# VishnoiAman777/FedRec-with-PytorchDistributed

Hardware: AMD Instinct MI355X
Metric: impressions/sec/node per FedAvg round + MIND AUC, 8 client-GPUs (higher is better)
Workload: dtype bf16

## Files before the change

### fedrec_with_pytorchdistributed_amd/csrc/bind_text_head.cpp

```cpp
#include "binding_util.h"

namespace {

int64_t head_titles(const at::Tensor& table, const OptTensor& ids, int64_t T) {
  check_dev(table, "table");
  TORCH_CHECK(table.dim() == 2 && table.is_contiguous() && table.scalar_type() == at::kBFloat16,
              "fedrec::head: table [rows, D] contiguous bf16");
  TORCH_CHECK(T >= 1 && table.size(0) % T == 0, "fedrec::head: table rows not a multiple of T");
  if (ids.has_value()) {
    check_dev(*ids, "ids");
    TORCH_CHECK(ids->dim() == 1 && ids->is_contiguous() && ids->scalar_type() == at::kInt, "fedrec::head: ids int32 [U]");
    return ids->size(0);
  }
  return table.size(0) / T;
}

Tensor2 head_score(const at::Tensor& table, const OptTensor& ids, int64_t T, const at::Tensor& w1, const at::Tensor& b1,
                   const at::Tensor& w2, const at::Tensor& b2, bool store_e, const OptTensor& nreal) {
  const int64_t U = head_titles(table, ids, T), D = table.size(1), Q = w1.size(0);
  check_dev(w1, "w1");
  TORCH_CHECK(w1.scalar_type() == at::kBFloat16 && w1.is_contiguous() && w1.size(1) == D, "fedrec::head_score: w1 bf16 [Q, D]");
  TORCH_CHECK(b1.scalar_type() == at::kFloat && w2.scalar_type() == at::kFloat && b2.scalar_type() == at::kFloat &&
                  b1.numel() == Q && w2.numel() == Q && b2.numel() == 1 && b1.is_contiguous() && w2.is_contiguous() &&
                  b1.is_cuda() && w2.is_cuda() && b2.is_cuda(),
              "fedrec::head_score: b1 / w2 [Q], b2 [1] fp32 device");
  TORCH_CHECK(fr_head_supported((int)D, (int)Q, (int)T), "fedrec::head_score: unsupported shape D=", D, " Q=", Q, " T=", T);
  const c10::DeviceGuard g(table.device());
  auto e = store_e ? at::empty({U * T, Q}, table.options()) : at::empty({0}, table.options());
  const int slices = fr_head_score_slices((int)Q);
  auto a = slices > 1 ? at::empty({slices, U * T}, table.options().dtype(at::kFloat))
                      : at::empty({U * T}, table.options().dtype(at::kFloat));
  check_rc(fr_head_score(table.data_ptr(), opt_int_ptr(ids), (int)U, (int)T, (int)D, (int)Q, w1.data_ptr(),
                         b1.data_ptr<float>(), w2.data_ptr<float>(), b2.data_ptr<float>(),
                         store_e ? e.data_ptr() : nullptr, a.data_ptr<float>(), opt_nreal(nreal, table), cur_stream()),
           "head_score");
  return {e, a};
}

Tensor3 head_pool(const at::Tensor& table, const OptTensor& ids, int64_t T, const at::Tensor& a, const OptTensor& tokens,
                  const OptTensor& nreal, bool want_bf16) {
  const int64_t U = head_titles(table, ids, T), D = table.size(1);
  check_dev(a, "a");
  TORCH_CHECK(a.scalar_type() == at::kFloat && (a.numel() == U * T || (a.dim() == 2 && a.size(0) == 2 && a.size(1) == U * T)) &&
                  a.is_contiguous(),
              "fedrec::head_pool: a [U*T] (or [2, U*T] score partials) fp32");
  if (tokens.has_value()) {
    check_dev(*tokens, "tokens");
    TORCH_CHECK(tokens->scalar_type() == at::kInt && tokens->dim() == 3 && tokens->size(1) == 2 &&
                    tokens->size(2) == T && tokens->is_contiguous() && tokens->size(0) * T >= table.size(0),
                "fedrec::head_pool: tokens int32 [N, 2, T] covering the table");
  }
  const c10::DeviceGuard g(table.device());
  auto pooled = at::empty({U, D}, a.options());
  auto alpha = at::empty({U, T}, a.options());
  auto pooled_b = at::empty({want_bf16 ? U : 0, D}, a.options().dtype(at::kBFloat16));
  check_rc(fr_head_pool(table.data_ptr(), opt_int_ptr(ids), a.data_ptr<float>(), a.dim() == 2 ? (int)a.size(0) : 1,
                        opt_int_ptr(tokens), (int)U, (int)T, (int)D, pooled.data_ptr<float>(), alpha.data_ptr<float>(),
                        opt_nreal(nreal, table), cur_stream(), want_bf16 ? pooled_b.data_ptr() : nullptr),
           "head_pool");
  return {pooled, alpha, pooled_b};
}

Tensor2 head_pool_bwd(const at::Tensor& table, const OptTensor& ids, int64_t T, const at::Tensor& alpha,
                      const at::Tensor& g, const OptTensor& nreal) {
  const int64_t U = head_titles(table, ids, T), D = table.size(1);
  check_dev(alpha, "alpha");
  check_dev(g, "g");
  TORCH_CHECK(alpha.scalar_type() == at::kFloat && alpha.numel() == U * T && alpha.is_contiguous() &&
                  g.scalar_type() == at::kFloat && g.numel() == U * D && g.is_contiguous(),
              "fedrec::head_pool_bwd: alpha [U, T], g [U, D] fp32");
  const c10::DeviceGuard dg(table.device());
  auto da = at::empty({U * T}, alpha.options());
  auto db2p = at::empty({std::max<int64_t>(U, 1)}, alpha.options());
  check_rc(fr_head_pool_bwd(table.data_ptr(), opt_int_ptr(ids), alpha.data_ptr<float>(), g.data_ptr<float>(), (int)U,
                            (int)T, (int)D, da.data_ptr<float>(), db2p.data_ptr<float>(), opt_nreal(nreal, table),
                            cur_stream()),
           "head_pool_bwd");
  return {da, db2p};
}

Tensor4 head_wgrad(const at::Tensor& table, const OptTensor& ids, int64_t T, const at::Tensor& e, const at::Tensor& da,
                   const at::Tensor& w2, const at::Tensor& db2p, const OptTensor& nreal) {
  const int64_t U = head_titles(table, ids, T), D = table.size(1), Q = w2.numel();
  check_dev(e, "e");
  check_dev(da, "da");
  check_dev(w2, "w2");
  check_dev(db2p, "db2p");
  TORCH_CHECK(e.scalar_type() == at::kBFloat16 && e.is_contiguous() && e.numel() == U * T * Q,
              "fedrec::head_wgrad: e bf16 [U*T, Q]");
  TORCH_CHECK(da.scalar_type() == at::kFloat && da.numel() == U * T && w2.scalar_type() == at::kFloat &&
                  w2.is_contiguous() && db2p.scalar_type() == at::kFloat && db2p.numel() >= U,
              "fedrec::head_wgrad: da / w2 / db2p");
  TORCH_CHECK(fr_head_supported((int)D, (int)Q, (int)T), "fedrec::head_wgrad: unsupported shape");
  const c10::DeviceGuard g(table.device());
  auto fopt = da.options();
  auto dW1 = at::empty({Q, D}, fopt);
  auto small = at::empty({2 * Q + 1}, fopt);
  float* db1 = small.data_ptr<float>();
  float* dw2 = db1 + Q;
  float* db2 = dw2 + Q;
  auto run = [&](float* scratch, const int* nr) {
    return fr_head_wgrad(e.data_ptr(), table.data_ptr(), opt_int_ptr(ids), da.data_ptr<float>(), db2p.data_ptr<float>(),
                         w2.data_ptr<float>(), (int)U, (int)T, (int)D, (int)Q, dW1.data_ptr<float>(), db1, dw2, db2,
                         scratch, nr, cur_stream());
  };
  const long need = run(nullptr, nullptr);
  TORCH_CHECK(need > 0, "fedrec::head_wgrad: unsupported shape");
  auto scratch = at::empty({need}, fopt);
  check_rc((int)run(scratch.data_ptr<float>(), opt_nreal(nreal, table)), "head_wgrad");
  return {dW1, small.narrow(0, 0, Q), small.narrow(0, Q, Q), small.narrow(0, 2 * Q, 1)};
}

Tensor3 head_pool_bwd_g(const at::Tensor& table, const OptTensor& ids, int64_t T, const at::Tensor& alpha,
                        const at::Tensor& g, at::Tensor e, const OptTensor& nreal) {
  const int64_t U = head_titles(table, ids, T), D = table.size(1);
  check_dev(alpha, "alpha");
  check_dev(g, "g");
  check_dev(e, "e");
  TORCH_CHECK(alpha.scalar_type() == at::kFloat && alpha.numel() == U * T && alpha.is_contiguous() &&
                  g.scalar_type() == at::kFloat && g.numel() == U * D && g.is_contiguous(),
              "fedrec::head_pool_bwd_g: alpha [U, T], g [U, D] fp32");
  TORCH_CHECK(e.scalar_type() == at::kBFloat16 && e.is_contiguous() && U > 0 && e.numel() % (U * T) == 0,
              "fedrec::head_pool_bwd_g: e bf16 [U*T, Q]");
  const int64_t Q = U > 0 ? e.numel() / (U * T) : 0;
  TORCH_CHECK(fr_head_g_supported((int)D, (int)Q, (int)T), "fedrec::head_pool_bwd_g: unsupported shape");
  const c10::DeviceGuard dg(table.device());
  auto da = at::empty({U * T}, alpha.options());
  auto db2p = at::empty({std::max<int64_t>(U, 1)}, alpha.options());
// ... 167 lines not shown
```

### fedrec_with_pytorchdistributed_amd/csrc/launchers.h

```cpp
#pragma once
#include <hip/hip_runtime_api.h>

extern "C" {

void fr_gemm_set_variant(int v);
int fr_gemm_nt_bf16(const void* A, const void* W, const float* bias, const void* R, void* C, int M, int N, int K, int act,
                    int c_rows, hipStream_t s);
int fr_gemm_nt_bf16_split(const void* A, const void* W, const float* bias, void* C, int M, int N, int K, int c_rows,
                          const int* full_rows, int n_partial, hipStream_t s);
int fr_gemm_gelu_bwd_colpart(const void* A, const void* W, const void* Z, void* C, float* colpart, int M, int N, int K,
                             int c_rows, hipStream_t s);
int fr_gemm_nt_bf16_dual(const void* A, const void* W, const float* bias, void* C, void* Z, int M, int N, int K,
                         int c_rows, hipStream_t s);

long fr_wgrad_bf16(const void* dY, const void* X, float* C, float* scratch, int M, int N, int K, int accumulate,
                   hipStream_t s);

void fr_ln_set_wide(int v);
int fr_layer_norm_bf16(const void* x, const float* w, const float* b, void* y, int rows, int D, float eps,
                       const void* res, hipStream_t s);
int fr_layer_norm_scatter_bf16(const void* x, const float* w, const float* b, void* y, int rows, int D, float eps,
                               const void* res, const int* dst, hipStream_t s);
int fr_layer_norm_bwd_bf16(const void* x, const float* w, const void* dy, void* dx, float* dw, float* db, int rows, int D,
                           float eps, hipStream_t s, float* dxs, void* dxz, float pdrop, unsigned long long seed,
                           unsigned long long offset);
int fr_gelu_bf16(const void* z, const void* dh, void* out, long n, int bwd, hipStream_t s);
int fr_embed_ln_bf16(const int* tokens, const void* word, const void* pos, const float* w, const float* b, void* y,
                     int rows, int D, int T, float eps, hipStream_t s);
int fr_embed_ln_rows_bf16(const int* tokens, const int* src, const void* word, const void* pos, const float* w,
                          const float* b, void* y, int rows, int D, int T, float eps, hipStream_t s);

int fr_dropout_add_bf16(const void* h, const void* res, void* out, long n, float p, unsigned long long seed,
                        unsigned long long offset, hipStream_t s);

void fr_title_attn_set_waves(int w);
int fr_title_attention_bf16(const void* qkv, const int* mask, void* out, int n_titles, int T, int H, int D,
                            hipStream_t s);
int fr_title_attention_drop_bf16(const void* qkv, const int* mask, void* out, int n_titles, int T, int H, int D,
                                 float pdrop, unsigned long long seed, unsigned long long offset, hipStream_t s);
int fr_title_plan(const int* mask, int n, int T, int* rowmap, int* src, int* kv_start, int* kv_len, int* qstart,
                  int* n_kv, hipStream_t s);
int fr_title_attention_packed_bf16(const void* qkv, const int* rowmap, const int* kv_start, const int* kv_len,
                                   const int* qstart, void* out, int n_titles, int T, int H, int D, hipStream_t s);

void fr_title_attn_bwd_set_variant(int v);
int fr_title_attention_bwd_bf16(const void* qkv, const void* dout, const int* mask, void* dqkv, int n_titles, int T, int H,
                                int D, hipStream_t s);
int fr_title_attention_bwd_drop_bf16(const void* qkv, const void* dout, const int* mask, void* dqkv, int n_titles,
                                     int T, int H, int D, float pdrop, unsigned long long seed,
                                     unsigned long long offset, hipStream_t s);

int fr_title_attention_long_bf16(const void* qkv, const int* mask, void* out, int n_titles, int T, int H, int D,
                                 hipStream_t s);
int fr_title_attention_bwd_long_bf16(const void* qkv, const void* dout, const int* mask, void* dqkv, int n_titles,
                                     int T, int H, int D, hipStream_t s);

int fr_colsum_chunks();
int fr_colsum_bf16(const void* x, int M, int N, float* partial, float* out, hipStream_t s, int ld);
int fr_gelu_bwd_colsum_bf16(const void* df, const void* z, void* dz, int M, int N, float* partial, float* out,
                            hipStream_t s);
int fr_embed_grad_bf16(const void* dx, const int* sorted, const int* perm, int R, int D, float* dword, int* scratch,
                       hipStream_t s);

void fr_head_score_set_rows(int r);
void fr_head_score_set_ilv(int v);
void fr_head_wgrad_g_set_kt(int kt);
int fr_head_supported(int D, int Q, int T);
int fr_head_g_supported(int D, int Q, int T);
int fr_head_score_slices(int Q);
int fr_head_score(const void* table, const int* ids, int U, int T, int D, int Q, const void* W1, const float* b1,
                  const float* w2, const float* b2, void* e_out, float* a_out, const int* nreal, hipStream_t s);
int fr_head_pool(const void* table, const int* ids, const float* a, int slices, const int* tokens, int U, int T, int D,
                 float* pooled, float* alpha, const int* nreal, hipStream_t s, void* pooled_b);
int fr_head_pool_bwd(const void* table, const int* ids, const float* alpha, const float* g, int U, int T, int D,
                     float* da, float* db2p, const int* nreal, hipStream_t s);
long fr_head_wgrad(const void* e, const void* table, const int* ids, const float* da, const float* db2p,
                   const float* w2, int U, int T, int D, int Q, float* dW1, float* db1, float* dw2, float* db2,
                   float* scratch, const int* nreal, hipStream_t s);
int fr_head_pool_bwd_g(const void* table, const int* ids, const float* alpha, const float* g, int U, int T, int D,
                       int Q, float* da, float* db2p, void* e, float* cs, const int* nreal, hipStream_t s);
long fr_head_wgrad_g(const void* G, const void* table, const int* ids, const float* cs, const float* db2p,
                     const float* w2, int U, int T, int D, int Q, float* dW1, float* db1, float* dw2, float* db2,
                     float* scratch, const int* nreal, hipStream_t s, const void* pend, int pend_cblocks,
                     int pend_total);

int fr_additive_pool_fwd(const void* x, const void* e, const float* w2, const float* b2, float* out, float* alpha,
                         int n, int T, int D, int Q, int is_bf16, const int* keep, hipStream_t s);
int fr_additive_pool_rows(int T, int D, int Q, int is_bf16);
int fr_additive_pool_bwd(const void* x, const void* e, const float* alpha, const float* w2, const float* g, float* dx,
                         void* dpre, float* dw2, float* db2, float* dsum, int n, int T, int D, int Q, int R,
                         int is_bf16, hipStream_t s);
int fr_upool_bwd_da(const float* x, const float* e, const float* alpha, const float* w2, const float* g, float* dx,
                    float* dpre, float* da8, int n, int T, int D, int Q, hipStream_t s, void* dpre_b);

int fr_user_attn_fwd(const float* qkv, float* ctx, float* stats, int B, int H, int NH, int dk, const int* keep,
                     hipStream_t s, void* ctx_b);
int fr_user_qkv_attn_fwd(const void* xd, const void* W, const float* bias, int Din, float* qkv, float* ctx,
                         float* stats, int B, int H, int NH, int dk, const int* keep, hipStream_t s, void* ctx_b);
int fr_user_attn_bwd_dctx(const float* qkv, const float* stats, const float* dctx, void* dqkv, const void* dpre,
                          const void* w1t, int Qd, int B, int H, int NH, int dk, const int* keep, hipStream_t s);
int fr_user_attn_bwd(const float* qkv, const float* stats, const float* dctx, void* dqkv, int B, int H, int NH,
                     int dk, const int* keep, hipStream_t s, int out_bf16);

void fr_score_set_variant(int v);
int fr_score_ce(const float* cand, const float* user, float* loss, float* scores, float* dcand, float* duser, int B,
                int C, int D, int sigm, const int* ci, float* loss_total, hipStream_t s);
int fr_user_pool_score(const float* x, const float* e, const float* w2, const float* b2, const int* keep,
                       const float* cand, const int* ci, int B, int T, int D, int Q, int C, int sigm, float* lossb,
                       float* scores, float* dcand, float* loss_total, float* dctx, float* dpre, void* dpre_b,
                       float* da8, hipStream_t s);

void fr_segsum_set_variant(int v);
void fr_segsum_set_ldp_block(int v);
int fr_segsum_chunks(int R);
int fr_segment_sum_rows(const float* rows, const int* perm, const int* seg_ptr, const int* inv, float* out, int U, int D,
                        int R, float* scratch, hipStream_t s, int zero_empty);
int fr_segment_sum_rows_ldp(const float* rows, const int* perm, const int* seg_ptr, const int* inv, float* out, int U,
                            int D, int R, float* scratch, float clip, float noise_std, unsigned long long seed,
                            unsigned long long offset, const unsigned long long* dev_off, hipStream_t s);
int fr_ldp_rows(const float* rows, float* out, int R, int D, float clip, float noise_std, unsigned long long seed,
                unsigned long long offset, hipStream_t s, const unsigned long long* dev_off);

void fr_small_gemm_set_rd(int v);
void fr_small_gemm_set_defer(int on);
long fr_small_gemm(const void* const* ptrs, const int* ints, const float* floats, const unsigned long long* seeds,
                   const unsigned long long* dev_off, int n, float* scratch, int tile, hipStream_t s);
int fr_small_gemm_has_pending();
int fr_small_gemm_batch_bytes();
int fr_small_gemm_take_pending(void* dst, int dst_bytes, int* c_blocks, int* total);
int fr_small_gemm_flush_pending(hipStream_t s);
long fr_colsum_f32(const float* const* xs, float* const* outs, const int* ints, int n, float* part, hipStream_t s);
int fr_gather_dropout(const float* v, const int* idx, void* out, int out_bf16, int M, int K, float p,
                      unsigned long long seed, unsigned long long offset, const unsigned long long* dev_off,
                      hipStream_t s);

int fr_adam_flat(float* p, const float* g, float* m, float* v, void* plow, long n, float lr, float b1, float b2,
                 float omb1, float omb2, float eps, float bc1, float bc2, float grad_scale, hipStream_t s);
int fr_adam_dev(float* p, float* g, float* m, float* v, void* plow, long n, float lr, double b1, double b2, float omb1,
                float omb2, float eps, float grad_scale, const long long* step, const float* loss, float* ring,
                int ring_n, hipStream_t s, int nseg, const float* const* gsrc, const long* goff, const long* gn,
                const int* skip);
int fr_multi_cast(const float* const* src, void* const* dst, const long* n, const int* to_bf16, int nseg,
                  long long* bump, hipStream_t s, long long* bump2, const long* nsrc, const int* fill, int ntseg,
                  const float* const* tsrc, void* const* tdst, const int* tR, const int* tC, const int* tld);
int fr_multi_cast_t(const float* const* src, void* const* dst, const int* R, const int* C, const int* ld, int nseg,
                    hipStream_t s);

int fr_sample_batch(const int* rows, const int* pos, const long long* neg_ptr, const int* negs, const long long* his_ptr,
                    const int* his, int* cand, int* hout, int B, int npr, int H, int truncate, unsigned long long seed,
                    unsigned long long offset, int valid, hipStream_t s);
int fr_dedup(const int* ids, int R, int num_news, int* uniq, int* inv, int* perm, int* seg_ptr, int* u_count,
             hipStream_t s);
int fr_multi_copy(const int* const* src, int* const* dst, const long* nsrc, const long* ndst, const int* fill, int n,
                  hipStream_t s);

void fr_topk_set_splits(int s);
int fr_topk_splits(long B, long N);
int fr_topk_scores(const float* user, const float* table, const int* exclude, void* ws, float* scores, int* ids, long B,
                   long N, int D, long E, int k, int min_id, hipStream_t s);

int fr_secagg_mask(const float* x, int* out, long n, float scale, float clipv, const unsigned long long* seeds,
                   const int* signs, int npeers, unsigned long long round, hipStream_t s);
int fr_secagg_unmask(const int* x, float* out, long n, float inv_scale, hipStream_t s);
int fr_secagg_hist(const float* x, long n, unsigned* scratch, int* out, const unsigned long long* seeds,
                   const int* signs, int npeers, unsigned long long round, hipStream_t s);
int fr_secagg_mask_exact(const float* x, int* out, long n, const int* H, int W, const unsigned long long* seeds,
                         const int* signs, int npeers, unsigned long long round, hipStream_t s);
// ... 13 lines not shown
```

### fedrec_with_pytorchdistributed_amd/csrc/text_head.hip

```cpp
#include "common.h"
#include "launchers.h"
#include "gemm_batch.h"

#include <stdlib.h>
#include <string.h>

#include <algorithm>

namespace {

constexpr int MAXT = 128;

__device__ __forceinline__ float tanh_fast(float x) {
  const float e = __builtin_amdgcn_exp2f(x * 2.8853900817779268f);
  return 1.0f - 2.0f * __builtin_amdgcn_rcpf(1.0f + e);
}

__device__ __attribute__((aligned(16))) bf16 g_zero_row[512];
__device__ float g_zero_f32[64];

__device__ __forceinline__ const bf16* hrow(const bf16* __restrict__ table, const int* __restrict__ ids, int m, int T,
                                            int D) {
  const int u = m / T;
  const int t = m - u * T;
// ... 146 lines not shown
      }
      if constexpr (SW) {
        static_assert(QFW <= 8, "lgkmcnt staging");
        __builtin_amdgcn_s_setprio(1);
#pragma unroll
        for (int i = 0; i < QFW; ++i) {
          lgkm_tie_rt(QFW - 1 - i, wr[i]);
          if (i == 0) {
#pragma unroll
            for (int j = 0; j < RFW; ++j) asm volatile("" : "+v"(xr[j]));
          }
#pragma unroll
          for (int j = 0; j < RFW; ++j)
            acc[i][j] = __builtin_amdgcn_mfma_f32_16x16x32_bf16(__builtin_bit_cast(bf16x8, wr[i]),
                                                                __builtin_bit_cast(bf16x8, xr[j]), acc[i][j], 0, 0, 0);
          if constexpr (ILV) {
            const int pc_ = kk * QFW + i;
            if (pc_ < PPW && nxt) issue_one(pc_, nst, nk0);
          }
        }
        __builtin_amdgcn_s_setprio(0);
        continue;
      }
      asm volatile("s_waitcnt lgkmcnt(0)" ::: "memory");
#pragma unroll
      for (int j = 0; j < RFW; ++j) asm volatile("" : "+v"(xr[j]));
#pragma unroll
      for (int i = 0; i < QFW; ++i) asm volatile("" : "+v"(wr[i]));
      __builtin_amdgcn_s_setprio(1);
#pragma unroll
      for (int i = 0; i < QFW; ++i)
#pragma unroll
        for (int j = 0; j < RFW; ++j)
          acc[i][j] = __builtin_amdgcn_mfma_f32_16x16x32_bf16(__builtin_bit_cast(bf16x8, wr[i]),
                                                              __builtin_bit_cast(bf16x8, xr[j]), acc[i][j], 0, 0, 0);
      __builtin_amdgcn_s_setprio(0);
    }
  }
  __syncthreads();

  float part[RFW];
#pragma unroll
  for (int j = 0; j < RFW; ++j) part[j] = 0.f;
#pragma unroll
  for (int i = 0; i < QFW; i += 2) {
    float v[2][RFW][4];
#pragma unroll
    for (int h = 0; h < 2; ++h) {
      const int qb = wq * QFW * 16 + (i + h) * 16 + fq * 4;
      const float4 bb = *(const float4*)(b1 + qb);
      const float4 ww = *(const float4*)(w2 + qb);
#pragma unroll
      for (int j = 0; j < RFW; ++j) {
        v[h][j][0] = tanh_fast(acc[i + h][j][0] + bb.x);
        v[h][j][1] = tanh_fast(acc[i + h][j][1] + bb.y);
        v[h][j][2] = tanh_fast(acc[i + h][j][2] + bb.z);
        v[h][j][3] = tanh_fast(acc[i + h][j][3] + bb.w);
        part[j] += v[h][j][0] * ww.x + v[h][j][1] * ww.y + v[h][j][2] * ww.z + v[h][j][3] * ww.w;
      }
    }
    if (e_out != nullptr) {
#pragma unroll
      for (int j = 0; j < RFW; ++j) {
        const int m = m0 + wm * 16 * RFW + j * 16 + fr;
        store_pair16_if(e_out + (size_t)(m < M ? m : 0) * ldq + wq * QFW * 16 + i * 16, v[0][j], v[1][j], fq, m < M);
      }
    }
  }
  float* red = (float*)smem;
#pragma unroll
  for (int j = 0; j < RFW; ++j) {
    const float s = group4_sum(part[j]);
    if (fq == 0) red[wq * MR + wm * 16 * RFW + j * 16 + fr] = s;
  }
  __syncthreads();
  if (tid < MR && m0 + tid < M) {
    float sa;
    if constexpr (WQ == 4) sa = (red[tid] + red[MR + tid]) + (red[2 * MR + tid] + red[3 * MR + tid]);
    else sa = red[tid] + red[MR + tid];
    a_out[m0 + tid] = sa + b2v;
  }
}

template <int TPT>
__global__ __launch_bounds__(384) void head_pool2_kernel(const bf16* __restrict__ table, const int* __restrict__ ids,
                                                         const float* __restrict__ a, const float* __restrict__ a2,
                                                         const int* __restrict__ tokens,
                                                         int T, int D, float* __restrict__ pooled,
                                                         float* __restrict__ alpha, const int* __restrict__ nreal,
                                                         bf16* __restrict__ pooled_b) {
  __shared__ float part[3072];
  const int u = blockIdx.x, tid = threadIdx.x, lane = tid & 63, wave = tid >> 6;
  if (nreal != nullptr && u >= nreal[0]) {
    for (int d = tid; d < D; d += blockDim.x) {
      pooled[(size_t)u * D + d] = 0.f;
      if (pooled_b != nullptr) pooled_b[(size_t)u * D + d] = f2bf(0.f);
    }
    for (int t = tid; t < T; t += blockDim.x) alpha[(size_t)u * T + t] = 0.f;
    return;
  }
  const int id = ids != nullptr ? ids[u] : u;
  const bf16* xe = table + (size_t)id * T * D;
  const int DC = D >> 3, TG = 384 / DC;
  const int dc = tid % DC, tgr = tid / DC;
  const int tg = tgr < TG ? tgr : TG - 1;
  bf16x8 v[TPT];
#pragma unroll
  for (int i = 0; i < TPT; ++i) {
    const int t = tg + TG * i;
    v[i] = *(const bf16x8*)(xe + (size_t)(t < T ? t : T - 1) * D + dc * 8);
  }
  float av[2], m = -INFINITY;
  bool keep[2];
#pragma unroll
  for (int c = 0; c < 2; ++c) {
    const int t = lane + 64 * c;
    keep[c] = t < T && (tokens == nullptr || tokens[((size_t)id * 2 + 1) * T + t] != 0);
    av[c] = keep[c] ? (a2 != nullptr ? a[(size_t)u * T + t] + a2[(size_t)u * T + t] : a[(size_t)u * T + t]) : -INFINITY;
    m = fmaxf(m, av[c]);
  }
  m = wave_max(m);
  if (!(m > -INFINITY)) m = 0.f;
  float p[2], l = 0.f;
#pragma unroll
  for (int c = 0; c < 2; ++c) {
    p[c] = keep[c] ? __expf(av[c] - m) : 0.f;
    l += p[c];
  }
  const float inv = 1.0f / (wave_sum(l) + 1e-8f * __expf(-m));
  const float al0 = p[0] * inv, al1 = p[1] * inv;
  if (wave == 0) {
    if (lane < T) alpha[(size_t)u * T + lane] = al0;
    if (lane + 64 < T) alpha[(size_t)u * T + lane + 64] = al1;
  }
  float acc[8] = {0.f, 0.f, 0.f, 0.f, 0.f, 0.f, 0.f, 0.f};
#pragma unroll
  for (int i = 0; i < TPT; ++i) {
    const int t = tg + TG * i;
    const float w0 = __shfl(al0, t & 63, 64), w1 = __shfl(al1, t & 63, 64);
    const float w = t < T ? (t < 64 ? w0 : w1) : 0.f;
    if (t < T) {
#pragma unroll
      for (int k = 0; k < 8; ++k) acc[k] += w * (float)v[i][k];
    }
  }
  if (tgr < TG) {
#pragma unroll
    for (int k = 0; k < 8; ++k) part[tg * D + dc * 8 + k] = acc[k];
  }
  __syncthreads();
  for (int d = tid; d < D; d += 384) {
    float s = 0.f;
    for (int j = 0; j < TG; ++j) s += part[j * D + d];
    pooled[(size_t)u * D + d] = s;
    if (pooled_b != nullptr) pooled_b[(size_t)u * D + d] = f2bf(s);
  }
}

template <int TPW>
__global__ __launch_bounds__(384) void head_pool_bwd2_kernel(const bf16* __restrict__ table,
                                                             const int* __restrict__ ids,
                                                             const float* __restrict__ alpha,
                                                             const float* __restrict__ g, int T, int D,
                                                             float* __restrict__ da, float* __restrict__ db2p,
                                                             const int* __restrict__ nreal) {
  __shared__ float dal[MAXT];
  const int u = blockIdx.x, tid = threadIdx.x, lane = tid & 63, wave = tid >> 6;
  if (nreal != nullptr && u >= nreal[0]) {
    for (int t = tid; t < T; t += blockDim.x) da[(size_t)u * T + t] = 0.f;
    if (tid == 0) db2p[u] = 0.f;
    return;
  }
  const int id = ids != nullptr ? ids[u] : u;
  const bf16* xe = table + (size_t)id * T * D;
  const float* gu = g + (size_t)u * D;
  const int DC = D >> 3;
  bf16x8 v[TPW][2];
#pragma unroll
  for (int i = 0; i < TPW; ++i) {
    const int t = wave + 6 * i;
    const bf16* row = xe + (size_t)(t < T ? t : T - 1) * D;
#pragma unroll
    for (int c = 0; c < 2; ++c) {
      const int dc = lane + 64 * c;
      v[i][c] = *(const bf16x8*)(row + (dc < DC ? dc : 0) * 8);
    }
  }
  float gv[2][8];
#pragma unroll
  for (int c = 0; c < 2; ++c) {
    const int dc = lane + 64 * c;
    const float4 g0 = dc < DC ? *(const float4*)(gu + dc * 8) : make_float4(0.f, 0.f, 0.f, 0.f);
    const float4 g1 = dc < DC ? *(const float4*)(gu + dc * 8 + 4) : make_float4(0.f, 0.f, 0.f, 0.f);
    gv[c][0] = g0.x; gv[c][1] = g0.y; gv[c][2] = g0.z; gv[c][3] = g0.w;
    gv[c][4] = g1.x; gv[c][5] = g1.y; gv[c][6] = g1.z; gv[c][7] = g1.w;
  }
  float s[TPW];
#pragma unroll
  for (int i = 0; i < TPW; ++i) {
    s[i] = 0.f;
#pragma unroll
// ... 703 lines not shown
  for (int j = 0; j < 4; ++j) xo[j] = G_BYTES + tr_off_pitch(2 * GKT, r0, wk * 64 + j * 16, q, p);
#pragma unroll
  for (int i = 0; i < QF; ++i) yo[i] = tr_off_pitch(2 * GQT, r0, wq * QF * 16 + i * 16, q, p);
  for (int st = 0; st < nsteps; ++st) {
    const int left = nsteps - 1 - st;
    const int inflight = left < NSTAGE - 2 ? left : NSTAGE - 2;
    __builtin_amdgcn_sched_barrier(0);
    if (inflight >= 2) asm volatile("s_waitcnt vmcnt(8) lgkmcnt(0)\n\ts_barrier" ::: "memory");
    else if (inflight == 1) asm volatile("s_waitcnt vmcnt(4) lgkmcnt(0)\n\ts_barrier" ::: "memory");
    else asm volatile("s_waitcnt vmcnt(0) lgkmcnt(0)\n\ts_barrier" ::: "memory");
    __builtin_amdgcn_sched_barrier(0);
    const bool nxt = st + NSTAGE - 1 < nsteps;
    const int nbuf = (st + NSTAGE - 1) % NSTAGE;
    if (nxt) stage(nbuf, mb + (st + NSTAGE - 1) * WTM);
    const uint32_t base = lds0 + (st % NSTAGE) * GSTB;
    s16x4 xr[8];
#pragma unroll
    for (int j = 0; j < 4; ++j) tr_read2<4 * 2 * GKT>(base + xo[j], xr[2 * j], xr[2 * j + 1]);
    s16x4 yr[2][4];
    tr_read2<4 * 2 * GQT>(base + yo[0], yr[0][0], yr[0][1]);
    tr_read2<4 * 2 * GQT>(base + yo[1], yr[0][2], yr[0][3]);
    bf16x8 xb[4];
#pragma unroll
    for (int ip = 0; ip < QF / 2; ++ip) {
      const int cur = ip & 1;
      if (ip + 1 < QF / 2) {
        tr_read2<4 * 2 * GQT>(base + yo[2 * ip + 2], yr[cur ^ 1][0], yr[cur ^ 1][1]);
        tr_read2<4 * 2 * GQT>(base + yo[2 * ip + 3], yr[cur ^ 1][2], yr[cur ^ 1][3]);
        lgkm_tie4<4>(yr[cur]);
      } else {
        lgkm_tie4<0>(yr[cur]);
      }
      if (ip == 0) {
        asm volatile("" : "+v"(xr[0]), "+v"(xr[1]), "+v"(xr[2]), "+v"(xr[3]), "+v"(xr[4]), "+v"(xr[5]), "+v"(xr[6]),
                     "+v"(xr[7]));
#pragma unroll
        for (int j = 0; j < 4; ++j) xb[j] = join(xr[2 * j], xr[2 * j + 1]);
      }
      __builtin_amdgcn_sched_barrier(0);
      __builtin_amdgcn_s_setprio(1);
#pragma unroll
      for (int f = 0; f < 2; ++f) {
        const bf16x8 ya = join(yr[cur][2 * f], yr[cur][2 * f + 1]);
#pragma unroll
        for (int j = 0; j < 4; ++j)
          acc[2 * ip + f][j] = __builtin_amdgcn_mfma_f32_16x16x32_bf16(xb[j], ya, acc[2 * ip + f][j], 0, 0, 0);
      }
      __builtin_amdgcn_s_setprio(0);
      __builtin_amdgcn_sched_barrier(0);
    }
  }
  float* out = P + (size_t)s * Q * D;
#pragma unroll
  for (int i = 0; i < QF; ++i) {
    const int qq2 = wq * QF * 16 + i * 16 + (lane & 15);
#pragma unroll
    for (int j = 0; j < 4; ++j) {
      const int k = k0 + wk * 64 + j * 16 + 4 * g;
      *(f32x4*)(out + (size_t)qq2 * D + k) = acc[i][j];
    }
  }
  const int per = (2 * Q + tiles_k - 1) / tiles_k;
  const int c = kt * per + tid;
  if (tid < per && c < 2 * Q) {
    const int which = c / Q, qc = c - which * Q;
    const float* src = cs + ((size_t)which * U) * Q + qc;
    float a0 = 0.f, a1 = 0.f, a2 = 0.f, a3 = 0.f;
    int u = u_lo;
    for (; u + 3 < u_hi; u += 4) {
      a0 += src[(size_t)u * Q];
      a1 += src[(size_t)(u + 1) * Q];
      a2 += src[(size_t)(u + 2) * Q];
      a3 += src[(size_t)(u + 3) * Q];
    }
    for (; u < u_hi; ++u) a0 += src[(size_t)u * Q];
    (which == 0 ? dw2p : dsump)[(size_t)s * Q + qc] = (a0 + a1) + (a2 + a3);
  }
}

int g_cus = 0;
int g_score_ilv = 1;
int g_score_rows = 0;

}

extern "C" void fr_head_score_set_rows(int r) { g_score_rows = r; }
extern "C" void fr_head_score_set_ilv(int v) { g_score_ilv = v; }

extern "C" int fr_head_supported(int D, int Q, int T) {
  return D % 256 == 0 && D <= 1024 && (Q == 128 || Q == 256 || Q == 384) && T >= 1 && T <= MAXT &&
         (T + 384 / (D / 8) - 1) / (384 / (D / 8)) <= 32;
}

extern "C" int fr_head_score(const void* table, const int* ids, int U, int T, int D, int Q, const void* W1,
                             const float* b1, const float* w2, const float* b2, void* e_out, float* a_out,
                             const int* nreal, hipStream_t s) {
  if (!fr_head_supported(D, Q, T)) return 1;
  const int M = U * T;
  if (M == 0) return 0;
  if (Q == 384) {
    if (g_cus == 0) {
      int dev = 0;
      (void)hipGetDevice(&dev);
      (void)hipDeviceGetAttribute(&g_cus, hipDeviceAttributeMultiprocessorCount, dev);
      if (g_cus <= 0) g_cus = 256;
    }
    const long Me = nreal != nullptr ? std::max<long>((long)M - 64L * T, (long)T) : (long)M;
    const long rounds192 = ((Me + 191) / 192 + g_cus - 1) / g_cus, rounds160 = ((Me + 159) / 160 + g_cus - 1) / g_cus;
    const bool r160 = g_score_rows == 160 || (g_score_rows == 0 && rounds160 * (160 + 384) < rounds192 * (192 + 384));
#define LAUNCH_S2(RF_, IL_)                                                                                  \
  hipLaunchKernelGGL((head_score2_kernel<6, RF_, 64, 2, 4, true, IL_>), dim3((M + 32 * RF_ - 1) / (32 * RF_)),     \
                     dim3(512), 0, s, (const bf16*)table, ids, M, T, D, (const bf16*)W1, b1, w2, b2, (bf16*)e_out, \
                     a_out, Q, nreal)
    if (r160) {
      if (g_score_ilv) LAUNCH_S2(5, true);
      else LAUNCH_S2(5, false);
    } else {
      if (g_score_ilv) LAUNCH_S2(6, true);
      else LAUNCH_S2(6, false);
    }
#undef LAUNCH_S2
    return 0;
  }
  if (Q == 256)
    hipLaunchKernelGGL((head_score2_kernel<4, 4, 64, 2, 4, true>), dim3((M + 127) / 128), dim3(512), 0, s,
                       (const bf16*)table, ids, M, T, D, (const bf16*)W1, b1, w2, b2, (bf16*)e_out, a_out, Q, nreal);
  else
    hipLaunchKernelGGL((head_score2_kernel<2, 4, 64, 2, 4, true>), dim3((M + 127) / 128), dim3(512), 0, s,
                       (const bf16*)table, ids, M, T, D, (const bf16*)W1, b1, w2, b2, (bf16*)e_out, a_out, Q, nreal);
  return 0;
}

extern "C" int fr_head_score_slices(int Q) {
  (void)Q;
  return 1;
}

extern "C" int fr_head_pool(const void* table, const int* ids, const float* a, int slices, const int* tokens, int U,
                            int T, int D, float* pooled, float* alpha, const int* nreal, hipStream_t s,
                            void* pooled_b) {
  const float* a2 = slices == 2 ? a + (size_t)U * T : nullptr;
  if (T > MAXT || D % 8 != 0 || D / 8 > 384) return 1;
  if (U == 0) return 0;
  const int TG = 384 / (D / 8), tpt = (T + TG - 1) / TG;
  if (tpt > 32) return 1;
  {
#define LAUNCH_POOL2(N)                                                                                          \
  hipLaunchKernelGGL(head_pool2_kernel<N>, dim3(U), dim3(384), 0, s, (const bf16*)table, ids, a, a2, tokens, T, D, \
                     pooled, alpha, nreal, (bf16*)pooled_b)
    if (tpt <= 13) LAUNCH_POOL2(13);
    else if (tpt <= 16) LAUNCH_POOL2(16);
    else LAUNCH_POOL2(32);
#undef LAUNCH_POOL2
    return 0;
  }
  return 0;
}

extern "C" int fr_head_pool_bwd(const void* table, const int* ids, const float* alpha, const float* g, int U, int T,
                                int D, float* da, float* db2p, const int* nreal, hipStream_t s) {
  if (T > MAXT || D % 8 != 0 || D / 8 > 128) return 1;
  if (U == 0) return 0;
  const int tpw = (T + 5) / 6;
  {
#define LAUNCH_PBWD2(N)                                                                                           \
  hipLaunchKernelGGL(head_pool_bwd2_kernel<N>, dim3(U), dim3(384), 0, s, (const bf16*)table, ids, alpha, g, T, D, \
                     da, db2p, nreal)
    if (tpw <= 9) LAUNCH_PBWD2(9);
    else if (tpw <= 11) LAUNCH_PBWD2(11);
    else LAUNCH_PBWD2(22);
#undef LAUNCH_PBWD2
    return 0;
  }
  return 0;
}

extern "C" long fr_head_wgrad(const void* e, const void* table, const int* ids, const float* da, const float* db2p,
                              const float* w2, int U, int T, int D, int Q, float* dW1, float* db1, float* dw2,
                              float* db2, float* scratch, const int* nreal, hipStream_t s) {
  if (!fr_head_supported(D, Q, T)) return -1;
  const int M = U * T;
  if (g_cus == 0) {
    int dev = 0;
    (void)hipGetDevice(&dev);
    (void)hipDeviceGetAttribute(&g_cus, hipDeviceAttributeMultiprocessorCount, dev);
    if (g_cus <= 0) g_cus = 256;
  }
  const int tiles_k = D / WKT, ntiles = (Q / WQT) * tiles_k;
  int S = g_cus / ntiles;
  const int smax = (M + 8 * WTM - 1) / (8 * WTM);
  S = S < 1 ? 1 : (S > smax ? smax : S);
  if (S < 1) S = 1;
  int mchunk = ((M + S - 1) / S + WTM - 1) / WTM * WTM;
  if (mchunk < WTM) mchunk = WTM;
  const int cap = (MAX_SPLIT_TITLES - 2) * T / WTM * WTM;
  if (mchunk > cap) mchunk = cap < 64 ? 64 : cap / 64 * 64;
  S = (M + mchunk - 1) / mchunk;
  if (S < 1) S = 1;
  const long need = (long)S * Q * D + 2L * S * Q;
  if (scratch == nullptr) return need;
  float* P = scratch;
  float* dw2p = scratch + (long)S * Q * D;
  float* dsump = dw2p + (long)S * Q;
  if (M > 0) {
    hipLaunchKernelGGL((head_wgrad_kernel<4, true, true>), dim3(S * ntiles), dim3(512), 0, s, (const bf16*)e,
                       (const bf16*)table, ids, da, M, T, D, Q, P, dw2p, dsump, tiles_k, ntiles, mchunk, 0, nreal);
  } else {
    (void)hipMemsetAsync(scratch, 0, need * sizeof(float), s);
  }
  const long n4 = (long)Q * D / 4;
  const long blocks = (n4 + 63) / 64 + (Q + 63) / 64 + 1;
  hipLaunchKernelGGL(head_reduce_kernel<false>, dim3((unsigned)blocks), dim3(256), 0, s, (const f32x4*)P, dw2p,
                     dsump, db2p, w2, (f32x4*)dW1, db1, dw2, db2, S, Q, D, U, fr_sg::GemmBatch{}, 0, 0);
  return 0;
}

extern "C" int fr_head_g_supported(int D, int Q, int T) {
  return Q == GQT && D % GKT == 0 && D <= 1024 && T >= 1 && T <= MAXT && fr_head_supported(D, Q, T);
}

extern "C" int fr_head_pool_bwd_g(const void* table, const int* ids, const float* alpha, const float* g, int U, int T,
                                  int D, int Q, float* da, float* db2p, void* e, float* cs, const int* nreal,
                                  hipStream_t s) {
  if (!fr_head_g_supported(D, Q, T) || D / 8 > 128) return 1;
  if (U == 0) return 0;
  const int tpw = (T + 5) / 6;
  const int EG = 384 / (Q / 8), etp = (T + EG - 1) / EG;
  if (tpw > 22 || etp > 16) return 1;
#define LAUNCH_PBWD3(N, E)                                                                                         \
  hipLaunchKernelGGL((head_pool_bwd3_kernel<N, E>), dim3(U), dim3(384), 0, s, (const bf16*)table, ids, alpha, g, T, \
                     D, Q, da, db2p, (bf16*)e, cs, U, nreal)
  if (tpw <= 9 && etp <= 7) LAUNCH_PBWD3(9, 7);
// ... 54 lines not shown
```

Baseline: 113,600.

## Add Q-sliced persistent head-score kernel with W1 slice resident in LDS

Adds a head-score kernel that splits the 384 query columns into four 96-wide slices over blockIdx.y. Each block keeps its W1 slice in LDS and walks a contiguous range of rows with register-prefetched table loads. It is selected when the row count exceeds one 160-row round per CU. Each slice writes a partial score plane, with b2 in a fifth plane, and the pool kernel sums the five planes. The aim is to stop reloading W1 per tile and to balance large M across CUs, at the cost of reading the table four times and extra score-plane traffic. A standalone memory-inbound probe kernel is also added.

```diff
diff --git a/fedrec_with_pytorchdistributed_amd/csrc/bind_text_head.cpp b/fedrec_with_pytorchdistributed_amd/csrc/bind_text_head.cpp
--- a/fedrec_with_pytorchdistributed_amd/csrc/bind_text_head.cpp
+++ b/fedrec_with_pytorchdistributed_amd/csrc/bind_text_head.cpp
@@ -27,7 +27,7 @@
   TORCH_CHECK(fr_head_supported((int)D, (int)Q, (int)T), "fedrec::head_score: unsupported shape D=", D, " Q=", Q, " T=", T);
   const c10::DeviceGuard g(table.device());
   auto e = store_e ? at::empty({U * T, Q}, table.options()) : at::empty({0}, table.options());
-  const int slices = fr_head_score_slices((int)Q);
+  const int slices = fr_head_score_slices((int)U, (int)T, (int)D, (int)Q, nreal.has_value() ? 1 : 0);
   auto a = slices > 1 ? at::empty({slices, U * T}, table.options().dtype(at::kFloat))
                       : at::empty({U * T}, table.options().dtype(at::kFloat));
   check_rc(fr_head_score(table.data_ptr(), opt_int_ptr(ids), (int)U, (int)T, (int)D, (int)Q, w1.data_ptr(),
@@ -41,9 +41,9 @@
                   const OptTensor& nreal, bool want_bf16) {
   const int64_t U = head_titles(table, ids, T), D = table.size(1);
   check_dev(a, "a");
-  TORCH_CHECK(a.scalar_type() == at::kFloat && (a.numel() == U * T || (a.dim() == 2 && a.size(0) == 2 && a.size(1) == U * T)) &&
+  TORCH_CHECK(a.scalar_type() == at::kFloat && (a.numel() == U * T || (a.dim() == 2 && (a.size(0) == 2 || a.size(0) == 5) && a.size(1) == U * T)) &&
                   a.is_contiguous(),
-              "fedrec::head_pool: a [U*T] (or [2, U*T] score partials) fp32");
+              "fedrec::head_pool: a [U*T] (or [2 | 5, U*T] score planes) fp32");
   if (tokens.has_value()) {
     check_dev(*tokens, "tokens");
     TORCH_CHECK(tokens->scalar_type() == at::kInt && tokens->dim() == 3 && tokens->size(1) == 2 &&
diff --git a/fedrec_with_pytorchdistributed_amd/csrc/launchers.h b/fedrec_with_pytorchdistributed_amd/csrc/launchers.h
--- a/fedrec_with_pytorchdistributed_amd/csrc/launchers.h
+++ b/fedrec_with_pytorchdistributed_amd/csrc/launchers.h
@@ -67,7 +67,7 @@
 void fr_head_wgrad_g_set_kt(int kt);
 int fr_head_supported(int D, int Q, int T);
 int fr_head_g_supported(int D, int Q, int T);
-int fr_head_score_slices(int Q);
+int fr_head_score_slices(int U, int T, int D, int Q, int padded);
 int fr_head_score(const void* table, const int* ids, int U, int T, int D, int Q, const void* W1, const float* b1,
                   const float* w2, const float* b2, void* e_out, float* a_out, const int* nreal, hipStream_t s);
 int fr_head_pool(const void* table, const int* ids, const float* a, int slices, const int* tokens, int U, int T, int D,
@@ -83,6 +83,9 @@
                      const float* w2, int U, int T, int D, int Q, float* dW1, float* db1, float* dw2, float* db2,
                      float* scratch, const int* nreal, hipStream_t s, const void* pend, int pend_cblocks,
                      int pend_total);
+
+int fr_cu_inbound_probe(const void* buf, long rows, const int* ids, int nids, int mode, int iters, int blocks,
+                        unsigned* sink, long long* cycles, hipStream_t s);
 
 int fr_additive_pool_fwd(const void* x, const void* e, const float* w2, const float* b2, float* out, float* alpha,
                          int n, int T, int D, int Q, int is_bf16, const int* keep, hipStream_t s);
diff --git a/fedrec_with_pytorchdistributed_amd/csrc/probe.hip b/fedrec_with_pytorchdistributed_amd/csrc/probe.hip
--- /dev/null
+++ b/fedrec_with_pytorchdistributed_amd/csrc/probe.hip
@@ -0,0 +1,89 @@
+#include "common.h"
+#include "launchers.h"
+
+namespace {
+
+constexpr int ROWB = 1536, KSTEPS = ROWB / 64, P = 8;
+typedef unsigned u32x4_t __attribute__((ext_vector_type(4)));
+
+template <int MODE, bool PAIR = false>
+__global__ __launch_bounds__(512, 1) void cu_inbound_probe_kernel(const char* __restrict__ buf, unsigned rows,
+                                                                   const int* __restrict__ ids, unsigned nids,
+                                                                   int iters, unsigned* __restrict__ sink,
+                                                                   long long* __restrict__ cycles) {
+  __shared__ __attribute__((aligned(16))) char smem[8 * P * 1024];
+  const int tid = threadIdx.x, lane = tid & 63, wave = tid >> 6;
+  const unsigned fr = lane & 15, fq = lane >> 4;
+  const unsigned nw = gridDim.x * 8, gw = blockIdx.x * 8 + wave;
+  auto row_ptr = [&](unsigned g) {
+    if constexpr (MODE == 4) return buf + (size_t)((g * 16 + (lane >> 3)) % rows) * ROWB + (lane & 7) * 16;
+    const unsigned m = g * 16 + fr;
+    const unsigned r = MODE == 2 ? (unsigned)ids[m % nids] % rows : m % rows;
+    return buf + (size_t)r * ROWB + fq * 16;
+  };
+  __syncthreads();
+  const long long t0 = __builtin_readcyclecounter();
+  unsigned g = gw;
+  if constexpr (MODE == 0) {
+    for (int it = 0; it < iters; ++it, g += nw) {
+      const char* cur = row_ptr(g);
+#pragma unroll
+      for (int s = 0; s < KSTEPS; ++s) {
+        asm volatile("s_waitcnt vmcnt(7)" ::: "memory");
+        __builtin_amdgcn_global_load_lds(GLOBAL_PTR(const void, cur + s * 64),
+                                         LDS_PTR(void, smem + (wave * P + (s & (P - 1))) * 1024), 16, 0, 0);
+      }
+    }
+    asm volatile("s_waitcnt vmcnt(0)" ::: "memory");
+    __syncthreads();
+    if (((const unsigned*)smem)[tid] == 0x9e3779b9u) sink[0] = 1u;
+  } else {
+    u32x4_t xr[P], acc = {0u, 0u, 0u, 0u};
+    const char* cur = row_ptr(g);
+#pragma unroll
+    for (int s = 0; s < P; ++s) xr[s] = *(const u32x4_t*)(MODE == 4 ? cur + (s & 1) * 8 * ROWB + (s >> 1) * 128 : cur + s * 64);
+    for (int it = 0; it < iters; ++it) {
+      g += nw;
+      const char* nxt = row_ptr(g);
+#pragma unroll
+      for (int s = 0; s < KSTEPS; ++s) {
+        acc ^= xr[s & (P - 1)];
+        auto refill = [&](int q) {
+          const int n = q + P < KSTEPS ? q + P : q + P - KSTEPS;
+          const char* b = q + P < KSTEPS ? cur : nxt;
+          xr[q & (P - 1)] = *(const u32x4_t*)(MODE == 4 ? b + (n & 1) * 8 * ROWB + (n >> 1) * 128 : b + n * 64);
+        };
+        if constexpr (!PAIR) {
+          refill(s);
+        } else if (s & 1) {
+          refill(s - 1);
+          refill(s);
+        }
+        __builtin_amdgcn_sched_barrier(0);
+      }
+      cur = nxt;
+    }
+    if ((acc[0] ^ acc[1] ^ acc[2] ^ acc[3]) == 0x9e3779b9u) sink[0] = 1u;
+  }
+  __syncthreads();
+  if (tid == 0) cycles[blockIdx.x] = (long long)__builtin_readcyclecounter() - t0;
+}
+
+}
+
+extern "C" int fr_cu_inbound_probe(const void* buf, long rows, const int* ids, int nids, int mode, int iters,
+                                   int blocks, unsigned* sink, long long* cycles, hipStream_t s) {
+  if (rows < 1 || rows > 0x7fffffffL / 16 || iters < 1 || blocks < 1 || mode < 0 || mode > 4) return 1;
+  if (mode == 2 && (ids == nullptr || nids < 1)) return 1;
+  if (mode == 4 && rows % 16 != 0) return 1;
+#define LAUNCH_PROBE(M_, P_)                                                                                   \
+  hipLaunchKernelGGL((cu_inbound_probe_kernel<M_, P_>), dim3(blocks), dim3(512), 0, s, (const char*)buf,       \
+                     (unsigned)rows, ids, (unsigned)nids, iters, sink, cycles)
+  if (mode == 0) LAUNCH_PROBE(0, false);
+  else if (mode == 1) LAUNCH_PROBE(1, false);
+  else if (mode == 3) LAUNCH_PROBE(1, true);
+  else if (mode == 4) LAUNCH_PROBE(4, false);
+  else LAUNCH_PROBE(2, true);
+#undef LAUNCH_PROBE
+  return 0;
+}
diff --git a/fedrec_with_pytorchdistributed_amd/csrc/text_head.hip b/fedrec_with_pytorchdistributed_amd/csrc/text_head.hip
--- a/fedrec_with_pytorchdistributed_amd/csrc/text_head.hip
+++ b/fedrec_with_pytorchdistributed_amd/csrc/text_head.hip
@@ -252,13 +252,214 @@
   }
 }
 
+template <int N>
+struct hs_int {
+  static constexpr int value = N;
+};
+
+template <int D>
+__global__ __launch_bounds__(512, 1) void head_score_ws_kernel(const bf16* __restrict__ table, const int* __restrict__ ids,
+                                                               int M, int T, const bf16* __restrict__ W1,
+                                                               const float* __restrict__ b1, const float* __restrict__ w2,
+                                                               const float* __restrict__ b2, bf16* __restrict__ e_out,
+                                                               float* __restrict__ a_out, int ldq,
+                                                               const int* __restrict__ nreal) {
+  constexpr int QS = 96, NQF = QS / 16;
+  constexpr int RB = D * 2, CPR = D / 8;
+  constexpr int NG = D / 256, NKS = D / 32, P = 8;
+  static_assert(D % 256 == 0 && QS * RB + 2 * QS * 4 <= 160 * 1024, "the W1 slice must fit LDS");
+  __shared__ __attribute__((aligned(16))) char smem[QS * RB + 2 * QS * 4];
+  {
+    const int qs = blockIdx.y;
+    W1 += (size_t)qs * QS * D;
+    b1 += qs * QS;
+    w2 += qs * QS;
+    if (e_out != nullptr) e_out += qs * QS;
+    a_out += (size_t)qs * M;
+  }
+  const int tid = threadIdx.x, lane = tid & 63, wave = tid >> 6;
+  const int fr = lane & 15, fq = lane >> 4;
+  const int Mr = nreal != nullptr ? min(M, nreal[0] * T) : M;
+  const int n16 = (Mr + 15) >> 4, NW = (int)gridDim.x * 8, gw = (int)blockIdx.x * 8 + wave;
+  const int r0 = (int)((long long)gw * n16 / NW) * 16, rend = (int)((long long)(gw + 1) * n16 / NW) * 16;
+  const bool work = r0 < rend;
+  const float b2v = b2[0];
+
+  auto title_id = [&](int m, int& t) {
+    m = m < Mr ? m : Mr - 1;
+    const int u = m / T;
+    t = m - u * T;
+    return ids != nullptr ? ids[u] : u;
+  };
+  const int lrow = lane >> 2, lchk = lane & 3;
+  auto row_ptr = [&](int id, int t) { return table + ((size_t)id * T + t) * D + lchk * 8; };
+  auto frag_row = [&](int r, int j) { return r + (j == 1 && r + 16 < rend ? 16 : 0) + lrow; };
+  const int psrc = (fr * 4 + fq) * 4;
+  auto to_mfma = [&](const u32x4_t& v) {
+    u32x4_t o;
+#pragma unroll
+    for (int k = 0; k < 4; ++k) o[k] = (unsigned)__builtin_amdgcn_ds_bpermute(psrc, (int)v[k]);
+    return o;
+  };
+
+  u32x4_t xr[P][2];
+  const bf16* cur[2] = {g_zero_row, g_zero_row};
+  if (work) {
+#pragma unroll
+    for (int j = 0; j < 2; ++j) {
+      int t;
+      const int id = title_id(frag_row(r0, j), t);
+      cur[j] = row_ptr(id, t);
+    }
+#pragma unroll
+    for (int s = 0; s < P; ++s)
+#pragma unroll
+      for (int j = 0; j < 2; ++j) xr[s][j] = *(const u32x4_t*)(cur[j] + s * 32);
+  }
+  float* const sb = (float*)(smem + QS * RB);
+  {
+    constexpr int NFILL = QS * CPR / 512;
+    static_assert(NFILL * 512 == QS * CPR, "fill tiling");
+    u32x4_t wv[NFILL];
+#pragma unroll
+    for (int i = 0; i < NFILL; ++i) {
+      const int c = tid + 512 * i, r = c / CPR, cc = c - r * CPR;
+      wv[i] = *(const u32x4_t*)(W1 + (size_t)r * D + cc * 8);
+    }
+#pragma unroll
+    for (int i = 0; i < NFILL; ++i) {
+      const int c = tid + 512 * i, r = c / CPR, cc = c - r * CPR;
+      *(u32x4_t*)(smem + r * RB + ((cc ^ (r & 15)) << 4)) = wv[i];
+    }
+  }
+  if (tid < QS) {
+    sb[tid] = b1[tid];
+    sb[QS + tid] = w2[tid];
+  }
+  __syncthreads();
+  if (!work) return;
+
+  const char* wbase[2][4];
+#pragma unroll
+  for (int h = 0; h < 2; ++h)
+#pragma unroll
+    for (int sl = 0; sl < 4; ++sl) {
+      uint32_t o = (uint32_t)((h * 48 + fr) * RB + (((sl * 4 + fq) ^ fr) << 4));
+      asm volatile("" : "+v"(o));
+      wbase[h][sl] = smem + o;
+    }
+  auto wfrag = [&](int ks, int i) {
+    return *(const u32x4_t*)(wbase[i / 3][ks & 3] + (ks >> 2) * 256 + (i % 3) * 16 * RB);
+  };
+
+  auto chunk = [&](int r, auto nf_c) __attribute__((always_inline)) {
+    constexpr int NF = decltype(nf_c)::value;
+    const int rn = r + 16 * NF;
+    const bool more = rn < rend;
+    int idn[2], tn[2];
+#pragma unroll
+    for (int j = 0; j < 2; ++j) idn[j] = title_id(frag_row(more ? rn : r, j), tn[j]);
+
+    f32x4 acc[NQF][NF];
+#pragma unroll
+    for (int i = 0; i < NQF; ++i)
+#pragma unroll
+      for (int j = 0; j < NF; ++j) acc[i][j] = f32x4{0.f, 0.f, 0.f, 0.f};
+    u32x4_t wf[2][NQF];
+    u32x4_t xo[2][NF];
+#pragma unroll
+    for (int i = 0; i < NQF; ++i) wf[0][i] = wfrag(0, i);
+#pragma unroll
+    for (int j = 0; j < NF; ++j) xo[0][j] = to_mfma(xr[0][j]);
+#pragma unroll
+    for (int g = 0; g < NG; ++g) {
+      const bf16* pf[2];
+#pragma unroll
+      for (int j = 0; j < 2; ++j) {
+        if (g + 1 < NG) pf[j] = cur[j] + (g + 1) * 256;
+        else pf[j] = more ? row_ptr(idn[j], tn[j]) : (const bf16*)g_zero_row;
+      }
+#pragma unroll
+      for (int s = 0; s < P; ++s) {
+        const int ks = g * P + s;
+        if (ks + 1 < NKS) {
+#pragma unroll
+          for (int i = 0; i < NQF; ++i) wf[(s + 1) & 1][i] = wfrag(ks + 1, i);
+#pragma unroll
+          for (int j = 0; j < NF; ++j) xo[(s + 1) & 1][j] = to_mfma(xr[(s + 1) & (P - 1)][j]);
+        }
+        if ((s & 1) == 0) {
+#pragma unroll
+          for (int h = 0; h < 2; ++h)
+#pragma unroll
+            for (int j = 0; j < 2; ++j) xr[s + h][j] = *(const u32x4_t*)(pf[j] + (s + h) * 32);
+        }
+        __builtin_amdgcn_sched_barrier(0);
+#pragma unroll
+        for (int i = 0; i < NQF; ++i)
+#pragma unroll
+          for (int j = 0; j < NF; ++j)
+            acc[i][j] = __builtin_amdgcn_mfma_f32_16x16x32_bf16(__builtin_bit_cast(bf16x8, wf[s & 1][i]),
+                                                                __builtin_bit_cast(bf16x8, xo[s & 1][j]), acc[i][j], 0, 0, 0);
+        __builtin_amdgcn_sched_barrier(0);
+      }
+      if (g + 1 == NG) {
+        cur[0] = pf[0];
+        cur[1] = pf[1];
+      }
+    }
+
+    float part[NF];
+#pragma unroll
+    for (int j = 0; j < NF; ++j) part[j] = 0.f;
+#pragma unroll
+    for (int i = 0; i < NQF; i += 2) {
+      float v[2][NF][4];
+#pragma unroll
+      for (int h = 0; h < 2; ++h) {
+        const int qb = (i + h) * 16 + fq * 4;
+        const float4 bb = *(const float4*)(sb + qb);
+        const float4 ww = *(const float4*)(sb + QS + qb);
+#pragma unroll
+        for (int j = 0; j < NF; ++j) {
+          v[h][j][0] = tanh_fast(acc[i + h][j][0] + bb.x);
+          v[h][j][1] = tanh_fast(acc[i + h][j][1] + bb.y);
+          v[h][j][2] = tanh_fast(acc[i + h][j][2] + bb.z);
+          v[h][j][3] = tanh_fast(acc[i + h][j][3] + bb.w);
+          part[j] += v[h][j][0] * ww.x + v[h][j][1] * ww.y + v[h][j][2] * ww.z + v[h][j][3] * ww.w;
+        }
+      }
+      if (e_out != nullptr) {
+#pragma unroll
+        for (int j = 0; j < NF; ++j) {
+          const int m = r + j * 16 + fr;
+          store_pair16_if(e_out + (size_t)(m < Mr ? m : 0) * ldq + i * 16, v[0][j], v[1][j], fq, m < Mr);
+        }
+      }
+    }
+#pragma unroll
+    for (int j = 0; j < NF; ++j) {
+      const int m = r + j * 16 + fr;
+      const float sa = group4_sum(part[j]);
+      if (fq == 0 && m < Mr) {
+        a_out[m] = sa;
+        if (blockIdx.y == 3) a_out[(size_t)M + m] = b2v;
+      }
+    }
+  };
+
+  int r = r0;
+  for (; r + 32 <= rend; r += 32) chunk(r, hs_int<2>{});
+  if (r < rend) chunk(r, hs_int<1>{});
+}
+
 template <int TPT>
 __global__ __launch_bounds__(384) void head_pool2_kernel(const bf16* __restrict__ table, const int* __restrict__ ids,
                                                          const float* __restrict__ a, const float* __restrict__ a2,
                                                          const int* __restrict__ tokens,
                                                          int T, int D, float* __restrict__ pooled,
                                                          float* __restrict__ alpha, const int* __restrict__ nreal,
-                                                         bf16* __restrict__ pooled_b) {
+                                                         bf16* __restrict__ pooled_b, const float* __restrict__ a3) {
   __shared__ float part[3072];
   const int u = blockIdx.x, tid = threadIdx.x, lane = tid & 63, wave = tid >> 6;
   if (nreal != nullptr && u >= nreal[0]) {
@@ -286,7 +487,11 @@
   for (int c = 0; c < 2; ++c) {
     const int t = lane + 64 * c;
     keep[c] = t < T && (tokens == nullptr || tokens[((size_t)id * 2 + 1) * T + t] != 0);
-    av[c] = keep[c] ? (a2 != nullptr ? a[(size_t)u * T + t] + a2[(size_t)u * T + t] : a[(size_t)u * T + t]) : -INFINITY;
+    const size_t ix = (size_t)u * T + t, pl = (size_t)gridDim.x * T;
+    if (!keep[c]) av[c] = -INFINITY;
+    else if (a3 != nullptr) av[c] = ((a[ix] + a2[ix]) + (a3[ix] + a3[pl + ix])) + a3[2 * pl + ix];
+    else if (a2 != nullptr) av[c] = a[ix] + a2[ix];
+    else av[c] = a[ix];
     m = fmaxf(m, av[c]);
   }
   m = wave_max(m);
@@ -1156,6 +1361,25 @@
 int g_score_ilv = 1;
 int g_score_rows = 0;
 
+int head_cus() {
+  if (g_cus == 0) {
+    int dev = 0;
+    (void)hipGetDevice(&dev);
+    (void)hipDeviceGetAttribute(&g_cus, hipDeviceAttributeMultiprocessorCount, dev);
+    if (g_cus <= 0) g_cus = 256;
+  }
+  return g_cus;
+}
+
+long score_rows_est(int M, int T, bool padded) {
+  return padded ? std::max<long>((long)M - 64L * T, (long)T) : (long)M;
+}
+bool score_ws_pick(int M, int T, int D, int Q, bool padded) {
+  if (Q != 384 || D % 256 != 0 || D > 768 || g_score_rows == 160 || g_score_rows == 192) return false;
+  if (g_score_rows == 96) return true;
+  return (score_rows_est(M, T, padded) + 159) / 160 > head_cus();
+}
+
 }
 
 extern "C" void fr_head_score_set_rows(int r) { g_score_rows = r; }
@@ -1172,14 +1396,22 @@
   if (!fr_head_supported(D, Q, T)) return 1;
   const int M = U * T;
   if (M == 0) return 0;
+  if (score_ws_pick(M, T, D, Q, nreal != nullptr)) {
+    const int units = (M + 15) / 16;
+    int nb = std::max(8, head_cus() / 4 / 8 * 8);
+    nb = std::min(nb, (units + 63) / 64 * 8);
+#define LAUNCH_WS(D_)                                                                                           \
+  hipLaunchKernelGGL((head_score_ws_kernel<D_>), dim3(nb, 4), dim3(512), 0, s, (const bf16*)table, ids, M, T, \
+                     (const bf16*)W1, b1, w2, b2, (bf16*)e_out, a_out, Q, nreal)
+    if (D == 768) LAUNCH_WS(768);
+    else if (D == 512) LAUNCH_WS(512);
+    else LAUNCH_WS(256);
+#undef LAUNCH_WS
+    return 0;
+  }
   if (Q == 384) {
-    if (g_cus == 0) {
-      int dev = 0;
-      (void)hipGetDevice(&dev);
-      (void)hipDeviceGetAttribute(&g_cus, hipDeviceAttributeMultiprocessorCount, dev);
-      if (g_cus <= 0) g_cus = 256;
-    }
-    const long Me = nreal != nullptr ? std::max<long>((long)M - 64L * T, (long)T) : (long)M;
+    (void)head_cus();
+    const long Me = score_rows_est(M, T, nreal != nullptr);
     const long rounds192 = ((Me + 191) / 192 + g_cus - 1) / g_cus, rounds160 = ((Me + 159) / 160 + g_cus - 1) / g_cus;
     const bool r160 = g_score_rows == 160 || (g_score_rows == 0 && rounds160 * (160 + 384) < rounds192 * (192 + 384));
 #define LAUNCH_S2(RF_, IL_)                                                                                  \
@@ -1205,15 +1437,16 @@
   return 0;
 }
 
-extern "C" int fr_head_score_slices(int Q) {
-  (void)Q;
-  return 1;
+extern "C" int fr_head_score_slices(int U, int T, int D, int Q, int padded) {
+  return score_ws_pick(U * T, T, D, Q, padded != 0) ? 5 : 1;
 }
 
 extern "C" int fr_head_pool(const void* table, const int* ids, const float* a, int slices, const int* tokens, int U,
                             int T, int D, float* pooled, float* alpha, const int* nreal, hipStream_t s,
                             void* pooled_b) {
-  const float* a2 = slices == 2 ? a + (size_t)U * T : nullptr;
+  if (slices != 1 && slices != 2 && slices != 5) return 1;
+  const float* a2 = slices >= 2 ? a + (size_t)U * T : nullptr;
+  const float* a3 = slices == 5 ? a + 2 * (size_t)U * T : nullptr;
   if (T > MAXT || D % 8 != 0 || D / 8 > 384) return 1;
   if (U == 0) return 0;
   const int TG = 384 / (D / 8), tpt = (T + TG - 1) / TG;
@@ -1221,7 +1454,7 @@
   {
 #define LAUNCH_POOL2(N)                                                                                          \
   hipLaunchKernelGGL(head_pool2_kernel<N>, dim3(U), dim3(384), 0, s, (const bf16*)table, ids, a, a2, tokens, T, D, \
-                     pooled, alpha, nreal, (bf16*)pooled_b)
+                     pooled, alpha, nreal, (bf16*)pooled_b, a3)
     if (tpt <= 13) LAUNCH_POOL2(13);
     else if (tpt <= 16) LAUNCH_POOL2(16);
     else LAUNCH_POOL2(32);
```

Result: faster. 115,700 (median of 6 runs) (+1.9%).
